# fema-ffrd/gpras

Hardware: AMD Instinct MI355X
Metric: gp_fits_per_sec (higher is better)
Workload: dtype f64; 1 GPU; BASELINE configs[1] as the many-independent-cells workload: exact GP N=4096 d=8 RBF, fit F1 = kernel build + blocked fp64-MFMA Cholesky + alpha + LML, per cell; cells = y columns of one training set with per-cell hyperparameters (the reference's per-mode models); n_train=4096, d=8, kernel=RBF, collective=none (one process), launcher=single process

## Files before the change

### gpras_amd/_lib.py

```python

from __future__ import annotations

import ctypes as C
from pathlib import Path

import numpy as np

import os

LIB_PATH = Path(os.environ["GPRX_LIBRARY"]) if os.environ.get("GPRX_LIBRARY") else Path(__file__).resolve().parent / "libgprx.so"

GPRX_OK, GPRX_EINVAL, GPRX_ENOTPD, GPRX_EHIP, GPRX_ENOMEM, GPRX_ESTATE, GPRX_ERCCL, GPRX_ENOCONV = range(8)
UNIQUE_ID_BYTES = 128
TRAIN_VARIANCE, TRAIN_LENGTHSCALE, TRAIN_NOISE, TRAIN_Z = 1, 2, 4, 8
GEMM_C_LOWER, GEMM_A_LOWER, GEMM_A_UPPER, GEMM_B_LOWER, GEMM_B_UPPER = 1, 2, 4, 8, 16
REDUCE_LOGDET_QUAD, REDUCE_COL, REDUCE_ROWSQ_FINAL, REDUCE_ROW = range(4)

DISTANCE_FORMS = {"difference": 0, "expanded": 1}
KERNEL_IDS = {"RBF": 0, "Matern12": 1, "Matern32": 2, "Matern52": 3, "Exponential": 4}


class GprxLibraryError(RuntimeError):
    """libgprx.so is missing or unusable."""

# ... 142 lines not shown
    "gprx_al_clip_dev": (C.c_int, [_vp, _vp, _i64, _i64, _i64, _i64, _vp, _i64]),
    "gprx_al_timings": (C.c_int, [_vp, _dp]),
    "gprx_dg_create": (C.c_int, [C.c_int, C.POINTER(_vp)]),
    "gprx_dg_destroy": (C.c_int, [_vp]),
    "gprx_dg_last_error": (C.c_char_p, [_vp]),
    "gprx_dg_synchronize": (C.c_int, [_vp]),
    "gprx_dg_sort_u64_dev": (C.c_int, [_vp, _vp, _i64, _vp]),
    "gprx_dg_sort_abs_residual_dev": (C.c_int, [_vp, _vp, _vp, _i64, _vp]),
    "gprx_dg_sort_info": (C.c_int, [_vp, _ip, _dp]),
    "gprx_dg_gather_dev": (C.c_int, [_vp, _vp, _i64, _vp, _i64, _vp]),
    "gprx_dg_scatter_summary_dev": (C.c_int, [_vp, _vp, _vp, _i64, _vp]),
    "gprx_dg_detect_dev": (C.c_int, [_vp, _vp, _vp, _i64, _i64, _vp, _vp, _i64, C.c_double, C.c_int, _vp, C.POINTER(_i64)]),
    "gprx_ev_create": (C.c_int, [C.c_int, _i64, _i64, _i64, _vp, _vp, _vp, _vp, _vp, C.POINTER(_vp)]),
    "gprx_ev_create_empty": (C.c_int, [C.c_int, C.POINTER(_vp)]),
    "gprx_ev_destroy": (C.c_int, [_vp]),
    "gprx_ev_last_error": (C.c_char_p, [_vp]),
    "gprx_ev_synchronize": (C.c_int, [_vp]),
    "gprx_ev_maxima": (C.c_int, [_vp, _vp, _vp, _vp]),
    "gprx_ev_return_periods": (C.c_int, [_vp, _i64, _vp, _vp, _vp]),
    "gprx_ev_rp_eval": (C.c_int, [_vp, C.c_int, _vp, _i64, _vp]),
    "gprx_ev_cov": (C.c_int, [_vp, C.c_int, _vp, _vp]),
    "gprx_ev_eigh": (C.c_int, [_vp, _vp, _vp, _ip]),
    "gprx_ev_scores": (C.c_int, [_vp, C.c_int, C.c_int, _vp]),
    "gprx_ev_standardise": (C.c_int, [_vp, _vp]),
    "gprx_ev_farthest": (C.c_int, [_vp, _vp, _i64, C.c_int, _vp, _i64, _i64, _vp, _vp]),
    "gprx_ev_timings": (C.c_int, [_vp, _dp]),
    "gprx_metrics": (C.c_int, [C.c_int, _vp, _vp, _vp, _i64, _i64, C.c_int, C.c_double, _vp, _vp, _vp, C.POINTER(C.c_uint64)]),
    "gprx_metrics_dev": (C.c_int, [C.c_int, _vp, _vp, _vp, _i64, _i64, C.c_int, C.c_double, _vp, _vp, _vp, C.POINTER(C.c_uint64)]),
    "gprx_kmeans_pp": (C.c_int, [C.c_int, _vp, _i64, C.c_int, _vp, C.c_int, C.c_int, _i64, _vp, _vp]),
    "gprx_kmeans_lloyd": (C.c_int, [C.c_int, _vp, _i64, C.c_int, _vp, C.c_int, C.c_double, C.c_int, _vp, _ip, _ip]),
    "gprx_gather_rows": (C.c_int, [C.c_int, _vp, _i64, _i64, _vp, _vp]),
    "gprx_kmat": (C.c_int, [C.c_int, C.c_int, _vp, _i64, _vp, _i64, C.c_int, _vp, C.c_double, C.c_double, _vp, _i64, _i64, _i64, C.c_int]),
    "gprx_gemm": (C.c_int, [C.c_int, C.c_int, C.c_int, _i64, _i64, _i64, C.c_double, _vp, _i64, _vp, _i64, C.c_double, _vp, _i64, C.c_int, C.c_int]),
    "gprx_potrf": (C.c_int, [C.c_int, _vp, _i64, _i64, _i64, _vp, _ip]),
    "gprx_gemm_batched": (C.c_int, [C.c_int, C.c_int, C.c_int, _i64, _i64, _i64, C.c_double, _vp, _i64, _vp, _i64, C.c_double, _vp, _i64, C.c_int, C.c_int,
                                    C.c_int, _i64, _i64, _i64, C.c_int, _i64, _i64, _i64, _vp, C.c_int, _vp, _i64]),
    "gprx_gemm_splitk": (C.c_int, [C.c_int, C.c_int, C.c_int, _i64, _i64, _i64, C.c_double, _vp, _i64, _vp, _i64, C.c_double, _vp, _i64, _vp, C.c_int,
                                   C.c_int, _i64, _i64, _i64, _i64, _vp, C.c_int]),
    "gprx_trsv_lower": (C.c_int, [C.c_int, _vp, _i64, _vp, _vp, _i64, C.c_int, C.c_int, _i64, _vp]),
    "gprx_potrf_batched": (C.c_int, [C.c_int, _vp, _i64, _i64, _i64, _vp, _vp, _vp, C.c_int, _i64, C.c_int, C.c_int, C.c_int, C.c_int, C.c_int, _ip]),
    "gprx_trsm_lower_left": (C.c_int, [C.c_int, _vp, _i64, _vp, _vp, _i64, _i64, _i64, C.c_int, _i64, _vp]),
    "gprx_trtri_lower": (C.c_int, [C.c_int, _vp, _i64, _vp, _vp, _i64, _vp, _i64, _i64, C.c_int, _i64, _i64, C.c_int]),
    "gprx_transpose_inplace": (C.c_int, [C.c_int, _vp, _i64, _i64, C.c_int, _i64]),
    "gprx_alpha_from_inverse": (C.c_int, [C.c_int, _vp, _i64, _vp, _vp, _vp, _i64, C.c_int, _i64, _i64, _i64]),
    "gprx_reduce_probe": (C.c_int, [C.c_int, C.c_int, _vp, _i64, _vp, _i64, _i64, C.c_double, C.c_double, C.c_int, _vp, C.c_int, _vp, C.c_int, _i64, _i64,
                                    _i64, _i64, _vp, _vp, C.c_int]),
    "gprx_set_tuning": (C.c_int, [C.c_char_p, C.c_int]),
    "gprx_set_handle_tuning": (C.c_int, [_vp, C.c_char_p, C.c_int]),
    "gprx_mfma_f64_peak": (C.c_int, [C.c_int, _dp]),
    "gprx_exp_probe": (C.c_int, [C.c_int, C.c_int, _vp, _i64, _vp]),
}

TUNING_KEYS = (
    "outer_block", "update_tile", "no_lookahead", "split_panel", "dag", "rhs_vector", "cell_kernel", "poison_workspace", "predict_path",
    "sgpr_fused", "sgpr_resident", "wait_handover_us", "sgpr_groups_from", "loeo_blocked_potrf",
    "held_general",
    "pcafit_rowsplit",
)
PCAFIT_ROUTES = ("gram", "covariance")

_lib = None


def load():
    global _lib
    if _lib is not None:
        return _lib
    if not LIB_PATH.exists():
        raise GprxLibraryError(
            f"{LIB_PATH} not found: build it with `python -c 'import __graft_entry__ as g; g.build()'` "
            "(hipcc --offload-arch=gfx950).  gpras_amd has no CPU fallback."
        )
    try:
        lib = C.CDLL(str(LIB_PATH))
    except OSError as exc:
        raise GprxLibraryError(f"cannot load {LIB_PATH}: {exc}") from exc
    for name, (res, args) in PROTOTYPES.items():
        try:
            fn = getattr(lib, name)
        except AttributeError as exc:
            raise GprxLibraryError(f"{LIB_PATH} does not export {name}") from exc
        fn.restype = res
        fn.argtypes = args
    _lib = lib
    return lib


def last_error(handle=None) -> str:
    msg = load().gprx_last_error(handle)
    return msg.decode() if msg else ""


def check(rc: int, handle=None) -> None:
    if rc == GPRX_OK:
        return
    msg = last_error(handle)
    if rc == GPRX_EINVAL:
        raise ValueError(msg)
    if rc == GPRX_ENOTPD:
        raise np.linalg.LinAlgError(msg)
    if rc == GPRX_ENOCONV:
        raise np.linalg.LinAlgError(msg)
    if rc == GPRX_ENOMEM:
        raise MemoryError(msg)
    raise RuntimeError(f"libgprx error {rc}: {msg}")


# ... 44 lines not shown
```

### gpras_amd/csrc/gprx.hip

```cpp
#include "abi_common.h"

#include <algorithm>
#include <chrono>
#include <cmath>
#include <cstdio>
#include <cstdlib>
#include <cstring>
#include <limits>
#include <map>
#include <mutex>
#include <string>
#include <thread>
#include <vector>

#include "gemm_f64.h"
#include "gprx_common.h"
#include "grad.h"
#include "kmat.h"
#include "potrf.h"
#include "potrf_cell.h"
#include "potrf_dag.h"
#include "sgpr.h"
#include "sgpr_asm.h"
#include "sgpr_fused.h"
// ... 622 lines not shown
  });
}

int gprx_trsm_lower_left(int device, const double* l_dev, int64_t lda, const double* inv_diag_dev, double* b_dev, int64_t ldb, int64_t n,
                         int64_t ncols, int cells, int64_t cs, const double* src_dev) {
  return guarded(nullptr, [&]() -> int {
    if (const char* why = solve_probe_invalid(l_dev, lda, inv_diag_dev, n, cells, cs)) return fail(nullptr, GPRX_EINVAL, why);
    if (!b_dev || off16(b_dev) || (src_dev && off16(src_dev))) return fail(nullptr, GPRX_EINVAL, "right-hand side must be given, 16-byte aligned");
    if (ncols <= 0 || ncols > (1 << 30) || ldb < ncols || odd(ldb)) return fail(nullptr, GPRX_EINVAL, "ldb must be even and at least ncols");
    if (src_dev && n != NB) return fail(nullptr, GPRX_EINVAL, "src is for n == 64 only");
    HIPCHK(nullptr, hipSetDevice(device));
    HIPCHK(nullptr, trsm_lower_left(util_stream(), l_dev, lda, inv_diag_dev, b_dev, ldb, (int)n, (int)ncols, cells, cs, src_dev));
    HIPCHK(nullptr, hipStreamSynchronize(util_stream()));
    return GPRX_OK;
  });
}

int gprx_trtri_lower(int device, const double* l_dev, int64_t lda, const double* inv_diag_dev, double* x_dev, int64_t ldx, double* t_dev,
                     int64_t ldt, int64_t np, int cells, int64_t cs_l, int64_t cs_x, int tile) {
  return guarded(nullptr, [&]() -> int {
    if (const char* why = solve_probe_invalid(l_dev, lda, inv_diag_dev, np, cells, cs_l)) return fail(nullptr, GPRX_EINVAL, why);
    if (!x_dev || !t_dev || off16(x_dev) || off16(t_dev)) return fail(nullptr, GPRX_EINVAL, "X and T must be given, 16-byte aligned");
    if (ldx < np || ldt < np || odd(ldx) || odd(ldt) || odd(cs_x) || cs_x < 0) return fail(nullptr, GPRX_EINVAL, "ldx, ldt, cs_x must be even, rows at least np");
    if (tile != 0 && tile != 64 && tile != 128) return fail(nullptr, GPRX_EINVAL, "tile must be 0, 64 or 128");
    HIPCHK(nullptr, hipSetDevice(device));
    HIPCHK(nullptr, trtri_lower(util_stream(), l_dev, lda, inv_diag_dev, x_dev, ldx, t_dev, ldt, (int)np, cells, cs_l, cs_x, tile));
    HIPCHK(nullptr, hipStreamSynchronize(util_stream()));
    return GPRX_OK;
  });
}

int gprx_potrf_batched(int device, double* a_dev, int64_t lda, int64_t np, int64_t extra, double* inv_diag_dev, double* stage_dev,
                       double* yvec_dev, int batch, int64_t cs, int route, int outer_block, int update_tile, int lookahead, int col_base,
                       int* info_host) {
  return guarded(nullptr, [&]() -> int {
    if (!a_dev || !inv_diag_dev || !stage_dev || !info_host) return fail(nullptr, GPRX_EINVAL, "null argument");
    if (np <= 0 || np % NB) return fail(nullptr, GPRX_EINVAL, "np must be a positive multiple of 64");
    if (extra < 0 || np > (1 << 30) || extra > (1 << 30)) return fail(nullptr, GPRX_EINVAL, "extra must not be negative, np and extra at most 2^30");
    if (lda < np || odd(lda) || odd(cs) || cs < 0) return fail(nullptr, GPRX_EINVAL, "lda and cs must be even, lda at least np");
    if (batch > 1 && cs < lda * (np + extra)) return fail(nullptr, GPRX_EINVAL, "cs shorter than one cell's matrix: the cells would overlap");
    if (off16(a_dev) || off16(inv_diag_dev) || off16(stage_dev) || (yvec_dev && off16(yvec_dev)))
      return fail(nullptr, GPRX_EINVAL, "operands must be 16-byte aligned");
    if (batch < 1 || route < 0 || route > 2 || col_base < 0) return fail(nullptr, GPRX_EINVAL, "batch must be positive, route 0, 1 or 2");
    if (yvec_dev && (route != 1 || batch == 1 || extra != 0))
      return fail(nullptr, GPRX_EINVAL, "the vector right-hand side is the split panel's, for batched cells without right-hand-side rows");
    if (route == 2 && extra % NB) return fail(nullptr, GPRX_EINVAL, "the cell kernel takes right-hand-side rows in tiles of 64");
    if (lookahead != 0 && (lookahead != 1 || batch > 1 || route == 2)) return fail(nullptr, GPRX_EINVAL, "look-ahead is for one matrix on routes 0 and 1");
    if (outer_block < 0 || outer_block % NB || (update_tile != 0 && update_tile != 64 && update_tile != 128))
      return fail(nullptr, GPRX_EINVAL, "outer_block must be a multiple of 64, update_tile 0, 64 or 128");
    PotrfTuning tune;
    tune.outer_block = outer_block;
    tune.update_tile = update_tile;
    tune.split_panel = route == 1 ? 1 : -1;
    HIPCHK(nullptr, hipSetDevice(device));
    hipStream_t st = util_stream();
    int* dinfo = nullptr;
    HIPCHK(nullptr, hipMalloc((void**)&dinfo, sizeof(int) * batch));
    hipError_t e = memset_sync(dinfo, 0, sizeof(int) * batch);
    PotrfStreams ps;
    if (e == hipSuccess && lookahead) e = ps.init();
    if (e == hipSuccess)
      e = route == 2 ? potrf_cells(st, a_dev, lda, (int)np, (int)extra, inv_diag_dev, dinfo, batch, cs, 1, col_base)
                     : potrf_lower(st, a_dev, lda, (int)np, (int)extra, inv_diag_dev, dinfo, stage_dev, nullptr, lookahead ? &ps : nullptr, batch, cs, 1,
                                   &tune, col_base, yvec_dev);
    hipError_t e2 = hipStreamSynchronize(st);
    if (ps.aux && e2 == hipSuccess) e2 = hipStreamSynchronize(ps.aux);
    ps.destroy();
    if (e == hipSuccess && e2 == hipSuccess) e2 = copy_sync(info_host, dinfo, sizeof(int) * batch, hipMemcpyDeviceToHost);
    hipFree(dinfo);
    HIPCHK(nullptr, e);
    HIPCHK(nullptr, e2);
    for (int c = 0; c < batch; ++c)
      if (info_host[c]) return fail(nullptr, GPRX_ENOTPD, "matrix not positive definite");
    return GPRX_OK;
  });
}

int gprx_transpose_inplace(int device, double* x_dev, int64_t ld, int64_t n, int cells, int64_t cs) {
  return guarded(nullptr, [&]() -> int {
    if (!x_dev || off16(x_dev)) return fail(nullptr, GPRX_EINVAL, "X must be given, 16-byte aligned");
    if (n <= 0 || n % 64 || n > (1 << 30) || ld < n || odd(ld) || cells < 1 || odd(cs) || cs < 0)
      return fail(nullptr, GPRX_EINVAL, "n must be a positive multiple of 64, ld and cs even");
    HIPCHK(nullptr, hipSetDevice(device));
    HIPCHK(nullptr, transpose_inplace(util_stream(), x_dev, ld, (int)n, cells, cs));
    HIPCHK(nullptr, hipStreamSynchronize(util_stream()));
    return GPRX_OK;
  });
}

int gprx_alpha_from_inverse(int device, const double* x_dev, int64_t ldx, const double* beta_dev, double* part_dev, double* alpha_dev, int64_t np,
                            int cells, int64_t cs_x, int64_t cs_b, int64_t cs_a) {
  return guarded(nullptr, [&]() -> int {
    if (!x_dev || !beta_dev || !part_dev || !alpha_dev) return fail(nullptr, GPRX_EINVAL, "null argument");
    if (np <= 0 || np % NB || np > (1 << 30) || ldx < np || cells < 1 || cs_x < 0 || cs_b < 0 || cs_a < 0)
      return fail(nullptr, GPRX_EINVAL, "np must be a positive multiple of 64");
    HIPCHK(nullptr, hipSetDevice(device));
    HIPCHK(nullptr, alpha_from_inverse(util_stream(), x_dev, ldx, beta_dev, part_dev, alpha_dev, (int)np, cells, cs_x, cs_b, cs_a));
    HIPCHK(nullptr, hipStreamSynchronize(util_stream()));
    return GPRX_OK;
  });
}

int gprx_reduce_probe(int device, int op, const double* m_dev, int64_t ldm, const double* w_dev, int64_t nrows, int64_t ncols, double base,
                      double scale, int accumulate, double* partial_dev, int rows_per_chunk, double* out_dev, int cells, int64_t m_cell,
                      int64_t w_cell, int64_t p_cell, int64_t out_cell, const double* base_tab_dev, const double* base_tab2_dev, int base_stride) {
  return guarded(nullptr, [&]() -> int {
// ... 64 lines not shown
int gprx_panel_acc(unsigned long long* out8, int reset) {
  if (reset) {
    unsigned long long z[8] = {0};
    hipMemcpyToSymbol(HIP_SYMBOL(gprx::g_panel_acc), z, sizeof(z));
  }
  hipMemcpyFromSymbol(out8, HIP_SYMBOL(gprx::g_panel_acc), sizeof(unsigned long long) * 8);
  return 0;
}
#endif
#ifdef GPRX_CELL_ACC
int gprx_cell_acc(unsigned long long* out16, int reset) {
  if (reset) {
    unsigned long long z[16] = {0};
    hipMemcpyToSymbol(HIP_SYMBOL(gprx::g_cell_acc), z, sizeof(z));
  }
  hipMemcpyFromSymbol(out16, HIP_SYMBOL(gprx::g_cell_acc), sizeof(unsigned long long) * 16);
  return 0;
}
#endif
int gprx_sf_stamps(gprx_handle h, int enable, unsigned long long* out) {
  return guarded(h, [&]() -> int {
    if (!h) return fail(h, GPRX_EINVAL, "null handle");
    HIPCHK(h, hipSetDevice(h->device));
    HIPCHK(h, hipStreamSynchronize(h->stream));
    if (out && h->sf_stamps) HIPCHK(h, copy_sync(out, h->sf_stamps, sizeof(unsigned long long) * SF_STAMP_WORDS, hipMemcpyDeviceToHost));
    if (enable && !h->sf_stamps) {
      HIPCHK(h, hipMalloc((void**)&h->sf_stamps, sizeof(unsigned long long) * SF_STAMP_WORDS));
      HIPCHK(h, memset_sync(h->sf_stamps, 0, sizeof(unsigned long long) * SF_STAMP_WORDS));
      drop_graphs(h);
    } else if (!enable && h->sf_stamps) {
      HIPCHK(h, hipFree(h->sf_stamps));
      h->sf_stamps = nullptr;
      drop_graphs(h);
    }
    return GPRX_OK;
  });
}
#ifdef GPRX_PANEL_STAMPS
int gprx_panel_stamps(unsigned long long* out64) {
  hipMemcpyFromSymbol(out64, HIP_SYMBOL(gprx::g_panel_stamps), sizeof(unsigned long long) * 64);
  return 0;
}
#endif

namespace {
bool apply_tuning(PotrfTuning& t, int& predict_path, int& fused, int& resident, const std::string& k, int value) {
  if (k == "outer_block" && value >= 0 && value % 128 == 0) t.outer_block = value;
  else if (k == "update_tile" && (value == 0 || value == 64 || value == 128)) t.update_tile = value;
  else if (k == "no_lookahead") t.no_lookahead = value != 0;
  else if (k == "split_panel" && value >= -1 && value <= 1) t.split_panel = value;
  else if (k == "dag" && value >= -1 && value <= 1) t.dag = value;
  else if (k == "rhs_vector" && value >= -1 && value <= 1) t.rhs_vector = value;
  else if (k == "cell_kernel" && value >= -1 && value <= 1) t.cell_kernel = value;
  else if (k == "poison_workspace" && value >= 0 && value <= 1) t.poison_workspace = value;
  else if (k == "predict_path" && value >= 0 && value <= 2) predict_path = value;
  else if (k == "sgpr_fused" && value >= 0 && value <= 1) fused = value;
  else if (k == "sgpr_resident" && value >= 0 && value <= 1) resident = value;
  else if (k == "wait_handover_us" && value >= 0) wait_handover_us() = value;
  else if (k == "sgpr_groups_from" && value >= 0) sf_groups_from() = value;
  else if (k == "loeo_blocked_potrf" && value >= -1 && value <= 2) loeo_blocked_potrf_force() = value;
  else if (k == "pcafit_rowsplit" && value >= 0 && value <= 1) pcafit_rowsplit_tuning() = value;
  else return false;
  return true;
}
}

int gprx_set_tuning(const char* key, int value) {
  return guarded(nullptr, [&]() -> int {
    if (!key) return fail(nullptr, GPRX_EINVAL, "null key");
    if (!apply_tuning(potrf_tuning(), predict_path_tuning(), sgpr_fused_tuning(), sgpr_resident_tuning(), key, value)) return fail(nullptr, GPRX_EINVAL, "unknown tuning key or bad value");
    return GPRX_OK;
  });
}

int gprx_set_handle_tuning(gprx_handle h, const char* key, int value) {
  return guarded(h, [&]() -> int {
    if (!h || !key) return fail(h, GPRX_EINVAL, "null argument");
    const int fused_before = h->sgpr_fused;
    if (std::string(key) == "held_general") {
      if (value < 0 || value > 1) return fail(h, GPRX_EINVAL, "unknown tuning key or bad value");
      h->held_general = value;
    } else if (!apply_tuning(h->tune, h->predict_path, h->sgpr_fused, h->sgpr_resident, key, value)) {
      return fail(h, GPRX_EINVAL, "unknown tuning key or bad value");
    }
    if (hipSetDevice(h->device) == hipSuccess && hipStreamSynchronize(h->stream) == hipSuccess) drop_graphs(h);
    if (h->sgpr_fused != fused_before) {
      h->sarena_slots = 0;
      if (h->m != 0) h->factorized = false;
    }
    return GPRX_OK;
  });
}

int gprx_mfma_f64_peak(int device, double* tflops) {
  return guarded(nullptr, [&]() -> int {
    if (!tflops) return fail(nullptr, GPRX_EINVAL, "null argument");
    HIPCHK(nullptr, hipSetDevice(device));
    double* out = nullptr;
    HIPCHK(nullptr, hipMalloc((void**)&out, 64));
    hipEvent_t e0, e1;
    hipEventCreate(&e0);
    hipEventCreate(&e1);
    const int iters = 20000, blocks = 256 * 4;
    hipStream_t us = util_stream();
    hipLaunchKernelGGL(mfma_f64_peak_kernel, dim3(blocks), dim3(256), 0, us, out, 100);
    hipEventRecord(e0, us);
// ... 17 lines not shown
```

### gpras_amd/csrc/potrf.h

```cpp
#pragma once
#include <cstdlib>
#include <utility>
#include <vector>

#include "chain64.h"
#include "gemm_f64.h"
#include "gprx_common.h"

namespace gprx {

#ifdef GPRX_PANEL_ACC
__device__ unsigned long long g_panel_acc[8];
#define PACC_DECL unsigned long long pacc_prev_ = 0;
#define PACC(i)                                                                                                       \
  {                                                                                                                   \
    if ((i) == 5) __builtin_amdgcn_s_waitcnt(0);                                                                      \
    const unsigned long long t_ = __builtin_amdgcn_s_memtime();                                                       \
    if (threadIdx.x == 0 && blockIdx.x == 0 && blockIdx.y == 0 && gridDim.x > 2) {                                    \
      if ((i) > 0) atomicAdd(&g_panel_acc[i], t_ - pacc_prev_);                                                       \
      else atomicAdd(&g_panel_acc[0], 1ull);                                                                          \
    }                                                                                                                 \
    pacc_prev_ = t_;                                                                                                  \
  }
#else
// ... 99 lines not shown
  if constexpr (P == 1) { PSTAMP(13) }
  __syncthreads();
  if constexpr (P == 1) { PSTAMP(14) }
  if constexpr (C0 + 8 < NB) {
    constexpr int KT0 = (C0 + 8) / 16;
    double fa[RT][2], fb[4][2];
#pragma unroll
    for (int rt = 0; rt < RT; ++rt)
#pragma unroll
      for (int ks = 0; ks < 2; ++ks) fa[rt][ks] = -c.sX[(WROWS * c.wave + 16 * rt + c.r) * PSUB + 4 * ks + c.g];
#pragma unroll
    for (int kt = KT0; kt < 4; ++kt) {
      const int kk = kt * 16 + c.r;
#pragma unroll
      for (int ks = 0; ks < 2; ++ks) fb[kt][ks] = (kk >= C0 + 8) ? c.sX[kk * PSUB + 4 * ks + c.g] : 0.0;
    }
#pragma unroll
    for (int kt = KT0; kt < 4; ++kt)
#pragma unroll
      for (int rt = 0; rt < RT; ++rt) {
        acc[rt][kt] = __builtin_amdgcn_mfma_f64_16x16x4f64(fa[rt][0], fb[kt][0], acc[rt][kt], 0, 0, 0);
        acc[rt][kt] = __builtin_amdgcn_mfma_f64_16x16x4f64(fa[rt][1], fb[kt][1], acc[rt][kt], 0, 0, 0);
      }
  }
  if ((c.r >> 3) == HALF) {
#pragma unroll
    for (int rt = 0; rt < RT; ++rt)
#pragma unroll
      for (int q = 0; q < 4; ++q) acc[rt][KT][q] = c.sX[(WROWS * c.wave + 16 * rt + c.g + 4 * q) * PSUB + (c.r & 7)];
  }
  if constexpr (P == 1) { PSTAMP(15) }
}

__device__ __forceinline__ void flush_staged_block(const double* __restrict__ prev_stage, double* __restrict__ prev_dst, int64_t lda,
                                                   int prev_pw, int tid) {
  if (!prev_stage) return;
  const int chunks = prev_pw / 2;
  for (int e = tid; e < prev_pw * chunks; e += 256) {
    const int row = e / chunks, cc = e % chunks;
    *reinterpret_cast<d2*>(prev_dst + (int64_t)row * lda + 2 * cc) = *reinterpret_cast<const d2*>(prev_stage + row * prev_pw + 2 * cc);
  }
}

__global__ __launch_bounds__(256) void copy_block_kernel(const double* __restrict__ stage, double* __restrict__ dst, int64_t lda, int pw,
                                                         int64_t cs) {
  flush_staged_block(stage + (int64_t)blockIdx.x * cs, dst + (int64_t)blockIdx.x * cs, lda, pw, threadIdx.x);
}

template <bool FUSE_K64>
__global__ __launch_bounds__(256, 2) void potrf_panel_kernel(double* __restrict__ A, int64_t lda, int rows_below, int nchunks,
                                                          double* __restrict__ inv_diag, int* __restrict__ info, int col0,
                                                          double* __restrict__ stage_out, const double* __restrict__ prev_stage,
                                                          double* __restrict__ prev_dst, int prev_pw, int64_t cs, int info_stride,
                                                          double* __restrict__ yv) {
  constexpr int PWG_ROWS = PANEL_WG_ROWS;
  constexpr int PANEL_ROWS = PANEL_OWN_ROWS;
  constexpr int WROWS = 16 * RT;
#ifndef GPRX_PANEL_NO_SETPRIO
  __builtin_amdgcn_s_setprio(3);
#endif
  {
    const int64_t off = (int64_t)blockIdx.y * cs;
    A += off;
    inv_diag += off;
    stage_out += off;
    if (prev_stage) prev_stage += off;
    if (prev_dst) prev_dst += off;
    info += (int64_t)blockIdx.y * info_stride;
  }
  __shared__ __attribute__((aligned(16))) double sIn[PWG_ROWS * PSUB];
  __shared__ __attribute__((aligned(16))) double sX[PWG_ROWS * PSUB];
  PanelCtx c;
  c.sIn = sIn;
  c.sX = sX;
  c.inv_diag = inv_diag;
  c.tid = threadIdx.x;
  const int lane = c.tid & 63;
  c.wave = c.tid >> 6;
  c.g = lane >> 4;
  c.r = lane & 15;
  c.zero_above = c.tid < NB ? c.tid : (1 << 30);
  c.bad = 0;
  const bool last = (int)blockIdx.x == nchunks;
  c.rinv_out = last ? stage_out + NB * NB : nullptr;
  if (last) flush_staged_block(prev_stage, prev_dst, lda, prev_pw, c.tid);
  c.out = nullptr;
  c.ident = -1;
  if (c.tid < NB) {
    if (last) c.out = stage_out + c.tid * NB;
  } else if (c.tid < PWG_ROWS) {
    if (last && c.tid < 2 * NB) c.ident = c.tid - NB;
  }
  PSTAMP(0)
  PACC_DECL
  PACC(0)

  d4 acc[RT][4];
  {
    const double* rowp[RT][4];
    bool valid[RT][4];
#pragma unroll
    for (int rt = 0; rt < RT; ++rt)
#pragma unroll
      for (int q = 0; q < 4; ++q) {
        const int wrow = WROWS * c.wave + 16 * rt + c.g + 4 * q;
        const int idx = (int)blockIdx.x * PANEL_ROWS + (wrow - NB);
        const bool diag = wrow < NB;
// ... 64 lines not shown
        const int wrow = WROWS * c.wave + 16 * rt + c.g + 4 * q;
#pragma unroll
        for (int kt = 0; kt < 4; ++kt) {
          const int col = kt * 16 + c.r;
          double v = valid[rt][q] ? acc[rt][kt][q] : 0.0;
          if (wrow < NB) {
            v = (col > wrow) ? 0.0 : v;
          } else if (last) {
            v = (col == wrow - NB) ? 1.0 : 0.0;
          }
          acc[rt][kt][q] = v;
        }
      }
  }
  PSTAMP(1)
  PACC(1)

  panel_step<0>(acc, c);
  PSTAMP(2)
  PACC(2)
  panel_step<1>(acc, c);
  panel_step<2>(acc, c);
  panel_step<3>(acc, c);
  PSTAMP(3)
  PACC(3)
  panel_step<4>(acc, c);
  panel_step<5>(acc, c);
  panel_step<6>(acc, c);
  panel_step<7>(acc, c);
  PSTAMP(4)
  PACC(4)
  if (!last) {
#pragma unroll
    for (int rt = 0; rt < RT; ++rt)
#pragma unroll
      for (int q = 0; q < 4; ++q) {
        const int wrow = WROWS * c.wave + 16 * rt + c.g + 4 * q;
        const int idx = (int)blockIdx.x * PANEL_ROWS + (wrow - NB);
        if (wrow >= NB && idx < rows_below) {
          double* dst = A + (int64_t)(NB + idx) * lda + c.r;
#pragma unroll
          for (int kt = 0; kt < 4; ++kt) dst[kt * 16] = acc[rt][kt][q];
        }
      }
  }
  if (last && c.tid == 0 && c.bad != 0) atomicCAS(info, 0, col0 + c.bad);
  if (yv != nullptr && last) {
    yv += (int64_t)blockIdx.y * cs;
    asm volatile("s_waitcnt vmcnt(0)" ::: "memory");
    __syncthreads();
    double* sv = sIn;
    double* sred = sIn + NB;
    static_assert(PWG_ROWS * PSUB >= NB + 256, "the sub-panel buffer holds y_j and the partial sums");
    if (c.tid < NB) sv[c.tid] = yv[c.tid];
    __syncthreads();
    const int a = c.tid & 63, qq = c.tid >> 6;
    const double* row = inv_diag + a * NB + 16 * qq;
    double sum = 0.0;
#pragma unroll
    for (int i = 0; i < 16; ++i) sum = __builtin_fma(row[i], sv[16 * qq + i], sum);
    sred[c.tid] = sum;
    __syncthreads();
    if (c.tid < NB) yv[c.tid] = ((sred[c.tid] + sred[64 + c.tid]) + sred[128 + c.tid]) + sred[192 + c.tid];
  }
  PSTAMP(5)
  PACC(5)
}

constexpr int ROWS_WG = 64 * RT;
__device__ __forceinline__ void wave_sync_lds() {
  __builtin_amdgcn_fence(__ATOMIC_RELEASE, "wavefront");
  __builtin_amdgcn_wave_barrier();
  __builtin_amdgcn_fence(__ATOMIC_ACQUIRE, "wavefront");
}
template <int P>
__device__ __forceinline__ void rows_step(d4 (&acc)[RT][4], double* __restrict__ sIn, double* __restrict__ sX, int tid, int wave, int g, int r,
                                          const double* __restrict__ gstage) {
  constexpr int C0 = 8 * P;
  constexpr int KT = C0 / 16;
  constexpr int HALF = P & 1;
  constexpr int WROWS = 16 * RT;
  if ((r >> 3) == HALF) {
#pragma unroll
    for (int rt = 0; rt < RT; ++rt)
#pragma unroll
      for (int q = 0; q < 4; ++q) sIn[(WROWS * wave + 16 * rt + g + 4 * q) * PSUB + (r & 7)] = acc[rt][KT][q];
  }
  wave_sync_lds();
  const int srow = WROWS * wave + (tid & 63);
  if ((tid & 63) < WROWS) {
    double x[8];
#pragma unroll
    for (int k = 0; k < 8; ++k) {
      double t = sIn[srow * PSUB + k];
#pragma unroll
      for (int m = 0; m < k; ++m) t = __builtin_fma(-x[m], gstage[(C0 + k) * NB + C0 + m], t);
      x[k] = t * gstage[NB * NB + C0 + k];
    }
#pragma unroll
    for (int k = 0; k < 8; ++k) sX[srow * PSUB + k] = x[k];
  }
  wave_sync_lds();
  if constexpr (C0 + 8 < NB) {
    constexpr int KT0 = (C0 + 8) / 16;
    double fa[RT][2], fb[4][2];
#pragma unroll
    for (int rt = 0; rt < RT; ++rt)
#pragma unroll
      for (int ks = 0; ks < 2; ++ks) fa[rt][ks] = -sX[(WROWS * wave + 16 * rt + r) * PSUB + 4 * ks + g];
#pragma unroll
    for (int kt = KT0; kt < 4; ++kt) {
      const int kk = kt * 16 + r;
#pragma unroll
      for (int ks = 0; ks < 2; ++ks) fb[kt][ks] = (kk >= C0 + 8) ? gstage[kk * NB + C0 + 4 * ks + g] : 0.0;
    }
#pragma unroll
    for (int kt = KT0; kt < 4; ++kt)
#pragma unroll
      for (int rt = 0; rt < RT; ++rt) {
        acc[rt][kt] = __builtin_amdgcn_mfma_f64_16x16x4f64(fa[rt][0], fb[kt][0], acc[rt][kt], 0, 0, 0);
        acc[rt][kt] = __builtin_amdgcn_mfma_f64_16x16x4f64(fa[rt][1], fb[kt][1], acc[rt][kt], 0, 0, 0);
      }
  }
  if ((r >> 3) == HALF) {
#pragma unroll
    for (int rt = 0; rt < RT; ++rt)
#pragma unroll
      for (int q = 0; q < 4; ++q) acc[rt][KT][q] = sX[(WROWS * wave + 16 * rt + g + 4 * q) * PSUB + (r & 7)];
  }
}

template <bool FUSE_K64, bool YVEC>
__global__ __launch_bounds__(256, FUSE_K64 ? 2 : 4) void potrf_rows_kernel(double* __restrict__ A21, int64_t lda, int rows_below,
                                                                           const double* __restrict__ stage, int64_t cs, double* __restrict__ yv) {
  constexpr int WG_ROWS = ROWS_WG, WROWS = 16 * RT;
  __shared__ __attribute__((aligned(16))) double sIn[WG_ROWS * PSUB];
  __shared__ __attribute__((aligned(16))) double sX[WG_ROWS * PSUB];
  A21 += (int64_t)blockIdx.y * cs;
  stage += (int64_t)blockIdx.y * cs;
  const int tid = threadIdx.x, lane = tid & 63, wave = tid >> 6, g = lane >> 4, r = lane & 15;
  const int row0 = blockIdx.x * WG_ROWS;
  d4 acc[RT][4];
  {
    const double* rowp[RT][4];
    bool valid[RT][4];
#pragma unroll
    for (int rt = 0; rt < RT; ++rt)
#pragma unroll
      for (int q = 0; q < 4; ++q) {
        const int idx = row0 + WROWS * wave + 16 * rt + g + 4 * q;
        valid[rt][q] = idx < rows_below;
        rowp[rt][q] = A21 + (int64_t)(valid[rt][q] ? idx : 0) * lda + r;
      }
    d4 upd[FUSE_K64 ? RT : 1][4];
    if constexpr (FUSE_K64) {
#pragma unroll
      for (int rt = 0; rt < RT; ++rt)
#pragma unroll
        for (int kt = 0; kt < 4; ++kt) upd[rt][kt] = d4{0.0, 0.0, 0.0, 0.0};
      const double* arow[RT];
#pragma unroll
      for (int rt = 0; rt < RT; ++rt) {
        const int idx = row0 + WROWS * wave + 16 * rt + r;
        arow[rt] = A21 + (int64_t)(idx < rows_below ? idx : 0) * lda - NB + 4 * g;
      }
      const double* brow = A21 - (int64_t)NB * lda + (int64_t)r * lda - NB + 4 * g;
#pragma unroll
      for (int k0 = 0; k0 < NB; k0 += 16) {
        double fa[RT][4], fb[4][4];
#pragma unroll
        for (int rt = 0; rt < RT; ++rt) {
          const d2 lo = *reinterpret_cast<const d2*>(arow[rt] + k0), hi = *reinterpret_cast<const d2*>(arow[rt] + k0 + 2);
          fa[rt][0] = lo.x; fa[rt][1] = lo.y; fa[rt][2] = hi.x; fa[rt][3] = hi.y;
        }
#pragma unroll
        for (int kt = 0; kt < 4; ++kt) {
          const double* bp = brow + (int64_t)(16 * kt) * lda + k0;
          const d2 lo = *reinterpret_cast<const d2*>(bp), hi = *reinterpret_cast<const d2*>(bp + 2);
          fb[kt][0] = lo.x; fb[kt][1] = lo.y; fb[kt][2] = hi.x; fb[kt][3] = hi.y;
        }
#pragma unroll
        for (int j = 0; j < 4; ++j)
#pragma unroll
          for (int rt = 0; rt < RT; ++rt)
#pragma unroll
            for (int kt = 0; kt < 4; ++kt) upd[rt][kt] = __builtin_amdgcn_mfma_f64_16x16x4f64(fa[rt][j], fb[kt][j], upd[rt][kt], 0, 0, 0);
      }
    }
#pragma unroll
    for (int rt = 0; rt < RT; ++rt)
#pragma unroll
      for (int q = 0; q < 4; ++q)
#pragma unroll
        for (int kt = 0; kt < 4; ++kt) acc[rt][kt][q] = rowp[rt][q][kt * 16];
    if constexpr (FUSE_K64) {
#pragma unroll
      for (int rt = 0; rt < RT; ++rt)
#pragma unroll
        for (int kt = 0; kt < 4; ++kt)
#pragma unroll
          for (int q = 0; q < 4; ++q) {
            const double v = -1.0 * upd[rt][kt][q];
            acc[rt][kt][q] = __builtin_fma(1.0, acc[rt][kt][q], v);
          }
    }
#pragma unroll
    for (int rt = 0; rt < RT; ++rt)
#pragma unroll
      for (int q = 0; q < 4; ++q)
#pragma unroll
        for (int kt = 0; kt < 4; ++kt) acc[rt][kt][q] = valid[rt][q] ? acc[rt][kt][q] : 0.0;
  }
  rows_step<0>(acc, sIn, sX, tid, wave, g, r, stage);
  rows_step<1>(acc, sIn, sX, tid, wave, g, r, stage);
  rows_step<2>(acc, sIn, sX, tid, wave, g, r, stage);
  rows_step<3>(acc, sIn, sX, tid, wave, g, r, stage);
  rows_step<4>(acc, sIn, sX, tid, wave, g, r, stage);
  rows_step<5>(acc, sIn, sX, tid, wave, g, r, stage);
  double ybj[YVEC ? 4 : 1], yold[YVEC ? RT : 1][4];
  if constexpr (YVEC) {
    yv += (int64_t)blockIdx.y * cs;
#pragma unroll
    for (int kt = 0; kt < 4; ++kt) ybj[kt] = yv[16 * kt + r];
#pragma unroll
    for (int rt = 0; rt < RT; ++rt)
#pragma unroll
      for (int q = 0; q < 4; ++q) {
        const int idx = row0 + WROWS * wave + 16 * rt + g + 4 * q;
        yold[rt][q] = yv[NB + (idx < rows_below ? idx : 0)];
      }
  }
  rows_step<6>(acc, sIn, sX, tid, wave, g, r, stage);
  rows_step<7>(acc, sIn, sX, tid, wave, g, r, stage);
#pragma unroll
  for (int rt = 0; rt < RT; ++rt)
#pragma unroll
    for (int q = 0; q < 4; ++q) {
      const int idx = row0 + WROWS * wave + 16 * rt + g + 4 * q;
      if (idx < rows_below) {
        double* dst = A21 + (int64_t)idx * lda + r;
#pragma unroll
        for (int kt = 0; kt < 4; ++kt) dst[kt * 16] = acc[rt][kt][q];
      }
    }
  if constexpr (YVEC) {
#pragma unroll
    for (int rt = 0; rt < RT; ++rt)
#pragma unroll
      for (int q = 0; q < 4; ++q) {
        double sum = acc[rt][0][q] * ybj[0];
#pragma unroll
        for (int kt = 1; kt < 4; ++kt) sum = __builtin_fma(acc[rt][kt][q], ybj[kt], sum);
#pragma unroll
        for (int m = 1; m < 16; m <<= 1) sum += __shfl_xor(sum, m, 64);
        const int idx = row0 + WROWS * wave + 16 * rt + g + 4 * q;
        if (r == 0 && idx < rows_below) yv[NB + idx] = yold[rt][q] - sum;
      }
  }
}

constexpr int STAGE_LD = 129;

struct PotrfProfile {
  std::vector<hipEvent_t> pool;
  size_t used = 0;
  std::vector<std::pair<size_t, double>> gemm_marks;
  std::vector<std::pair<size_t, double>> strip_marks;
  std::vector<size_t> panel_marks;
  hipEvent_t next() {
    if (used == pool.size()) {
      hipEvent_t e;
      hipEventCreate(&e);
      pool.push_back(e);
    }
    return pool[used++];
  }
  void reset() {
    used = 0;
    gemm_marks.clear();
    strip_marks.clear();
    panel_marks.clear();
  }
  ~PotrfProfile() {
    for (auto e : pool) hipEventDestroy(e);
  }
};

struct PotrfTuning {
  int outer_block = 0;
  int update_tile = 0;
  int no_lookahead = 0;
  int split_panel = 0;
  int poison_workspace = 0;
  int cell_kernel = 0;
  int rhs_vector = 0;
  int dag = 0;
};
inline PotrfTuning& potrf_tuning() {
  static PotrfTuning t = [] {
    PotrfTuning v;
    if (const char* e = getenv("GPRX_OUTER_BLOCK")) v.outer_block = atoi(e);
    if (const char* e = getenv("GPRX_UPDATE_TILE")) v.update_tile = atoi(e);
    if (const char* e = getenv("GPRX_SPLIT_PANEL")) v.split_panel = atoi(e);
    if (const char* e = getenv("GPRX_DAG")) v.dag = atoi(e);
    if (const char* e = getenv("GPRX_RHS_VECTOR")) v.rhs_vector = atoi(e);
    if (const char* e = getenv("GPRX_CELL_KERNEL")) v.cell_kernel = atoi(e);
    return v;
  }();
  return t;
}

struct PotrfStreams {
  hipStream_t aux = nullptr;
  hipEvent_t block_done = nullptr, tail_done = nullptr;
  hipError_t init() {
    hipError_t e = hipStreamCreateWithFlags(&aux, hipStreamNonBlocking);
    if (e != hipSuccess) return e;
    if ((e = hipEventCreateWithFlags(&block_done, hipEventDisableTiming)) != hipSuccess) return e;
    return hipEventCreateWithFlags(&tail_done, hipEventDisableTiming);
  }
  void destroy() {
    if (aux) hipStreamDestroy(aux);
    if (block_done) hipEventDestroy(block_done);
    if (tail_done) hipEventDestroy(tail_done);
    aux = nullptr;
    block_done = tail_done = nullptr;
  }
};

inline bool potrf_split_panel(const PotrfTuning& tune, int batch) { return tune.split_panel ? tune.split_panel > 0 : batch >= 24; }

inline bool potrf_rhs_vector_ok(const PotrfTuning& tune, int batch) { return tune.rhs_vector >= 0 && batch > 1 && potrf_split_panel(tune, batch); }

inline hipError_t potrf_lower(hipStream_t st, double* A, int64_t lda, int np, int extra, double* inv_diag, int* info,
                              double* diag_stage, PotrfProfile* prof = nullptr, PotrfStreams* ps = nullptr, int batch = 1, int64_t cs = 0,
                              int info_stride = 0, const PotrfTuning* tune_in = nullptr, int col_base = 0, double* yvec = nullptr) {
  const double* prev_stage = nullptr;
  double* prev_dst = nullptr;
  auto mark_gemm = [&](hipStream_t s, int ncols_lower, int rows_rect, int ncols, int k, bool strip = false) {
    if (!prof) return;
    const double elems = 0.5 * (double)ncols_lower * (ncols_lower + 1) + (double)rows_rect * ncols;
    (strip ? prof->strip_marks : prof->gemm_marks).push_back({prof->used, 2.0 * k * elems * batch});
    hipEventRecord(prof->next(), s);
  };
  auto mark_end = [&](hipStream_t s) {
    if (prof) hipEventRecord(prof->next(), s);
  };
  const int total_rows = np + extra;
  const PotrfTuning& tune = tune_in ? *tune_in : potrf_tuning();
  if (tune.no_lookahead) ps = nullptr;
  const int ob = tune.outer_block ? tune.outer_block : (np > 4096 ? 512 : 1024);
  const int bulk_tile = tune.update_tile ? tune.update_tile : 64;
  bool tail_pending = false;
  hipError_t err = hipSuccess;
  const bool split_panel = potrf_split_panel(tune, batch);
  if (yvec && !split_panel) return hipErrorInvalidValue;
  auto panel = [&](int c, bool fuse = false) {
    const int rows_below = total_rows - c - NB;
    double* Acc = A + (int64_t)c * lda + c;
    if (prof) {
      prof->panel_marks.push_back(prof->used);
      hipEventRecord(prof->next(), st);
    }
    double* stage_out = diag_stage + (int64_t)c * STAGE_LD;
    double* invd = inv_diag + (int64_t)(c / NB) * NB * NB;
    double* yv = yvec ? yvec + c : nullptr;
    const int own_rows = split_panel ? 0 : rows_below;
    const int nchunks = (own_rows + PANEL_OWN_ROWS - 1) / PANEL_OWN_ROWS;
    const auto diag = fuse ? potrf_panel_kernel<true> : potrf_panel_kernel<false>;
    hipLaunchKernelGGL(diag, dim3(nchunks + 1, batch), dim3(256), 0, st, Acc, lda,
                       own_rows, nchunks, invd, info, col_base + c, stage_out, prev_stage, prev_dst, NB, cs, info_stride, yv);
    if (split_panel && rows_below > 0) {
      const auto rows = fuse ? (yv ? potrf_rows_kernel<true, true> : potrf_rows_kernel<true, false>)
                             : (yv ? potrf_rows_kernel<false, true> : potrf_rows_kernel<false, false>);
      hipLaunchKernelGGL(rows, dim3((rows_below + ROWS_WG - 1) / ROWS_WG, batch), dim3(256), 0, st, Acc + (int64_t)NB * lda, lda, rows_below,
                         (const double*)stage_out, cs, yv);
    }
    prev_stage = stage_out;
    prev_dst = Acc;
    if (prof) hipEventRecord(prof->next(), st);
  };
  auto update = [&](int c0, int k, int c1, int n, int tile) {
    const int rows = total_rows - c1;
    const double* L21 = A + (int64_t)c1 * lda + c0;
    double* A22 = A + (int64_t)c1 * lda + c1;
    mark_gemm(st, n, rows - n, n, k, k <= 128);
    hipError_t e = launch_gemm(st, 0, 1, rows, n, k, -1.0, L21, lda, L21, lda, 1.0, A22, lda, GEMM_C_LOWER, k == NB ? 64 : tile, batch, cs, cs, cs);
    mark_end(st);
    if (e != hipSuccess && err == hipSuccess) err = e;
  };
  auto factor_range = [&](auto&& self, int c0, int w) -> void {
    if (w <= NB) {
      panel(c0);
      return;
    }
    const int h = ((w / NB + 1) / 2) * NB;
    self(self, c0, h);
    if (h == NB && w - h == NB) {
      panel(c0 + h, true);
      return;
    }
    update(c0, h, c0 + h, w - h, 64);
    self(self, c0 + h, w - h);
  };
  for (int C = 0; C < np; C += ob) {
    const int w = (np - C < ob) ? np - C : ob;
    factor_range(factor_range, C, w);
    if (err != hipSuccess) return err;
    const int R = C + w;
    if (R >= np) break;
    const int wn = (np - R < ob) ? np - R : ob;
    if (ps && tail_pending) hipStreamWaitEvent(st, ps->tail_done, 0);
    update(C, w, R, wn, batch > 1 ? bulk_tile : 64);
    if (err != hipSuccess) return err;
    if (ps) hipEventRecord(ps->block_done, st);
    const int R2 = R + wn;
    if (R2 < np) {
      hipStream_t ts = ps ? ps->aux : st;
      if (ps) hipStreamWaitEvent(ts, ps->block_done, 0);
      const int rows = total_rows - R2, cols = np - R2;
      const double* Lrow = A + (int64_t)R2 * lda + C;
      mark_gemm(ts, cols, rows - cols, cols, w);
      hipError_t e = launch_gemm(ts, 0, 1, rows, cols, w, -1.0, Lrow, lda, Lrow, lda, 1.0, A + (int64_t)R2 * lda + R2, lda, GEMM_C_LOWER,
                                   bulk_tile, batch, cs, cs, cs);
      mark_end(ts);
      if (e != hipSuccess) return e;
      if (ps) {
        hipEventRecord(ps->tail_done, ts);
        tail_pending = true;
      }
    }
  }
  if (prev_stage) hipLaunchKernelGGL(copy_block_kernel, dim3(batch), dim3(256), 0, st, prev_stage, prev_dst, lda, NB, cs);
  if (ps && tail_pending) hipStreamWaitEvent(st, ps->tail_done, 0);
  return hipGetLastError();
}

}
```

Baseline: 2260 fits/s.

## Fuse paired 64-column panel row solves into one rows kernel pass

For batched split-panel Cholesky, two adjacent 64-wide panels are now handled by a paired rows kernel. It runs both triangular row solves in one launch and keeps the y-vector update in LDS between the passes. The first diagonal panel factors its own 64 rows so the second panel can apply the k=64 update, and the rows kernel is refactored into a reusable device function that uses buffer loads and non-temporal loads and stores. This is meant to cut kernel launches and global memory round trips per panel pair. The cost is heavier register pressure, a changed launch-bounds occupancy, and a more complex correctness path.

```diff
diff --git a/gpras_amd/_lib.py b/gpras_amd/_lib.py
--- a/gpras_amd/_lib.py
+++ b/gpras_amd/_lib.py
@@ -218,7 +218,7 @@
 }
 
 TUNING_KEYS = (
-    "outer_block", "update_tile", "no_lookahead", "split_panel", "dag", "rhs_vector", "cell_kernel", "poison_workspace", "predict_path",
+    "outer_block", "update_tile", "no_lookahead", "split_panel", "dag", "rhs_vector", "rows_pair", "cell_kernel", "poison_workspace", "predict_path",
     "sgpr_fused", "sgpr_resident", "wait_handover_us", "sgpr_groups_from", "loeo_blocked_potrf",
     "held_general",
     "pcafit_rowsplit",
diff --git a/gpras_amd/csrc/gprx.hip b/gpras_amd/csrc/gprx.hip
--- a/gpras_amd/csrc/gprx.hip
+++ b/gpras_amd/csrc/gprx.hip
@@ -698,6 +698,7 @@
     tune.outer_block = outer_block;
     tune.update_tile = update_tile;
     tune.split_panel = route == 1 ? 1 : -1;
+    tune.rows_pair = potrf_tuning().rows_pair;
     HIPCHK(nullptr, hipSetDevice(device));
     hipStream_t st = util_stream();
     int* dinfo = nullptr;
@@ -868,6 +869,7 @@
   else if (k == "dag" && value >= -1 && value <= 1) t.dag = value;
   else if (k == "rhs_vector" && value >= -1 && value <= 1) t.rhs_vector = value;
   else if (k == "cell_kernel" && value >= -1 && value <= 1) t.cell_kernel = value;
+  else if (k == "rows_pair" && value >= 0 && value <= 1) t.rows_pair = value;
   else if (k == "poison_workspace" && value >= 0 && value <= 1) t.poison_workspace = value;
   else if (k == "predict_path" && value >= 0 && value <= 2) predict_path = value;
   else if (k == "sgpr_fused" && value >= 0 && value <= 1) fused = value;
diff --git a/gpras_amd/csrc/potrf.h b/gpras_amd/csrc/potrf.h
--- a/gpras_amd/csrc/potrf.h
+++ b/gpras_amd/csrc/potrf.h
@@ -175,7 +175,7 @@
                                                           double* __restrict__ inv_diag, int* __restrict__ info, int col0,
                                                           double* __restrict__ stage_out, const double* __restrict__ prev_stage,
                                                           double* __restrict__ prev_dst, int prev_pw, int64_t cs, int info_stride,
-                                                          double* __restrict__ yv) {
+                                                          double* __restrict__ yv, int y_left) {
   constexpr int PWG_ROWS = PANEL_WG_ROWS;
   constexpr int PANEL_ROWS = PANEL_OWN_ROWS;
   constexpr int WROWS = 16 * RT;
@@ -346,9 +346,20 @@
     double* sv = sIn;
     double* sred = sIn + NB;
     static_assert(PWG_ROWS * PSUB >= NB + 256, "the sub-panel buffer holds y_j and the partial sums");
-    if (c.tid < NB) sv[c.tid] = yv[c.tid];
+    const int a = c.tid & 63, qq = c.tid >> 6;
+    if (FUSE_K64 && y_left) {
+      const double* brow = A + (int64_t)a * lda - NB + 16 * qq;
+      const double* bl = yv - NB + 16 * qq;
+      double sum = 0.0;
+#pragma unroll
+      for (int i = 0; i < 16; ++i) sum = __builtin_fma(brow[i], bl[i], sum);
+      sred[c.tid] = sum;
+      __syncthreads();
+      if (c.tid < NB) sv[c.tid] = yv[c.tid] - (((sred[c.tid] + sred[64 + c.tid]) + sred[128 + c.tid]) + sred[192 + c.tid]);
+    } else {
+      if (c.tid < NB) sv[c.tid] = yv[c.tid];
+    }
     __syncthreads();
-    const int a = c.tid & 63, qq = c.tid >> 6;
     const double* row = inv_diag + a * NB + 16 * qq;
     double sum = 0.0;
 #pragma unroll
@@ -424,27 +435,40 @@
   }
 }
 
-template <bool FUSE_K64, bool YVEC>
-__global__ __launch_bounds__(256, FUSE_K64 ? 2 : 4) void potrf_rows_kernel(double* __restrict__ A21, int64_t lda, int rows_below,
-                                                                           const double* __restrict__ stage, int64_t cs, double* __restrict__ yv) {
-  constexpr int WG_ROWS = ROWS_WG, WROWS = 16 * RT;
-  __shared__ __attribute__((aligned(16))) double sIn[WG_ROWS * PSUB];
-  __shared__ __attribute__((aligned(16))) double sX[WG_ROWS * PSUB];
-  A21 += (int64_t)blockIdx.y * cs;
-  stage += (int64_t)blockIdx.y * cs;
-  const int tid = threadIdx.x, lane = tid & 63, wave = tid >> 6, g = lane >> 4, r = lane & 15;
-  const int row0 = blockIdx.x * WG_ROWS;
+__device__ __forceinline__ d2 ld2_l2(__amdgpu_buffer_rsrc_t rs, unsigned voff, unsigned soff) {
+  typedef unsigned int u4v __attribute__((ext_vector_type(4)));
+  const u4v v = __builtin_amdgcn_raw_buffer_load_b128(rs, voff, soff, 16);
+  d2 out;
+  __builtin_memcpy(&out, &v, 16);
+  return out;
+}
+template <int M>
+__device__ __forceinline__ double lane_xor(double v) {
+  int w[2];
+  __builtin_memcpy(w, &v, 8);
+  w[0] = __builtin_amdgcn_ds_swizzle(w[0], (M << 10) | 0x1f);
+  w[1] = __builtin_amdgcn_ds_swizzle(w[1], (M << 10) | 0x1f);
+  __builtin_memcpy(&v, w, 8);
+  return v;
+}
+template <bool FUSE_K64, bool YVEC, bool X_L2, bool Y_IN, bool Y_OUT, bool NT_IN = false, bool NT_OUT = false>
+__device__ __forceinline__ void rows_pass(double* __restrict__ A21, int64_t lda, int rows_below, int row0, const double* __restrict__ stage,
+                                          double* __restrict__ yv, int64_t ycell, int ybeta, int yrows, double* __restrict__ sIn,
+                                          double* __restrict__ sX) {
+  constexpr int WROWS = 16 * RT;
+  const int lane = __lane_id(), wave = __builtin_amdgcn_readfirstlane(threadIdx.x >> 6), tid = 64 * wave + lane, g = lane >> 4, r = lane & 15;
   d4 acc[RT][4];
   {
-    const double* rowp[RT][4];
+    const char* wg0 = reinterpret_cast<const char*>(A21 + (int64_t)row0 * lda);
+    unsigned rowp[RT][4];
     bool valid[RT][4];
 #pragma unroll
     for (int rt = 0; rt < RT; ++rt)
 #pragma unroll
       for (int q = 0; q < 4; ++q) {
-        const int idx = row0 + WROWS * wave + 16 * rt + g + 4 * q;
-        valid[rt][q] = idx < rows_below;
-        rowp[rt][q] = A21 + (int64_t)(valid[rt][q] ? idx : 0) * lda + r;
+        const int lrow = WROWS * wave + 16 * rt + g + 4 * q;
+        valid[rt][q] = row0 + lrow < rows_below;
+        rowp[rt][q] = ((unsigned)(valid[rt][q] ? lrow : 0) * (unsigned)lda + r) * 8u;
       }
     d4 upd[FUSE_K64 ? RT : 1][4];
     if constexpr (FUSE_K64) {
@@ -453,10 +477,14 @@
 #pragma unroll
         for (int kt = 0; kt < 4; ++kt) upd[rt][kt] = d4{0.0, 0.0, 0.0, 0.0};
       const double* arow[RT];
+      [[maybe_unused]] __amdgpu_buffer_rsrc_t xrs;
+      [[maybe_unused]] unsigned xoff[RT];
+      if constexpr (X_L2) xrs = __builtin_amdgcn_make_buffer_rsrc(A21 + (int64_t)row0 * lda - NB, 0, 0xffffffff, 0x00020000);
 #pragma unroll
       for (int rt = 0; rt < RT; ++rt) {
         const int idx = row0 + WROWS * wave + 16 * rt + r;
         arow[rt] = A21 + (int64_t)(idx < rows_below ? idx : 0) * lda - NB + 4 * g;
+        if constexpr (X_L2) xoff[rt] = ((unsigned)(idx < rows_below ? idx - row0 : 0) * (unsigned)lda + 4u * g) * 8u;
       }
       const double* brow = A21 - (int64_t)NB * lda + (int64_t)r * lda - NB + 4 * g;
 #pragma unroll
@@ -464,7 +492,14 @@
         double fa[RT][4], fb[4][4];
 #pragma unroll
         for (int rt = 0; rt < RT; ++rt) {
-          const d2 lo = *reinterpret_cast<const d2*>(arow[rt] + k0), hi = *reinterpret_cast<const d2*>(arow[rt] + k0 + 2);
+          d2 lo, hi;
+          if constexpr (X_L2) {
+            lo = ld2_l2(xrs, xoff[rt], 8u * k0);
+            hi = ld2_l2(xrs, xoff[rt], 8u * k0 + 16u);
+          } else {
+            lo = *reinterpret_cast<const d2*>(arow[rt] + k0);
+            hi = *reinterpret_cast<const d2*>(arow[rt] + k0 + 2);
+          }
           fa[rt][0] = lo.x; fa[rt][1] = lo.y; fa[rt][2] = hi.x; fa[rt][3] = hi.y;
         }
 #pragma unroll
@@ -486,7 +521,10 @@
 #pragma unroll
       for (int q = 0; q < 4; ++q)
 #pragma unroll
-        for (int kt = 0; kt < 4; ++kt) acc[rt][kt][q] = rowp[rt][q][kt * 16];
+        for (int kt = 0; kt < 4; ++kt) {
+          const double* src = reinterpret_cast<const double*>(wg0 + rowp[rt][q] + kt * 128);
+          acc[rt][kt][q] = NT_IN ? __builtin_nontemporal_load(src) : *src;
+        }
     if constexpr (FUSE_K64) {
 #pragma unroll
       for (int rt = 0; rt < RT; ++rt)
@@ -512,16 +550,18 @@
   rows_step<4>(acc, sIn, sX, tid, wave, g, r, stage);
   rows_step<5>(acc, sIn, sX, tid, wave, g, r, stage);
   double ybj[YVEC ? 4 : 1], yold[YVEC ? RT : 1][4];
+  [[maybe_unused]] int yrow0 = row0;
   if constexpr (YVEC) {
-    yv += (int64_t)blockIdx.y * cs;
-#pragma unroll
-    for (int kt = 0; kt < 4; ++kt) ybj[kt] = yv[16 * kt + r];
+    yv += ycell;
+    asm volatile("" : "+s"(yrow0));
+#pragma unroll
+    for (int kt = 0; kt < 4; ++kt) ybj[kt] = yv[ybeta + 16 * kt + r];
 #pragma unroll
     for (int rt = 0; rt < RT; ++rt)
 #pragma unroll
       for (int q = 0; q < 4; ++q) {
-        const int idx = row0 + WROWS * wave + 16 * rt + g + 4 * q;
-        yold[rt][q] = yv[NB + (idx < rows_below ? idx : 0)];
+        const int idx = yrow0 + WROWS * wave + 16 * rt + g + 4 * q;
+        yold[rt][q] = Y_IN ? sIn[(WROWS * wave + 16 * rt + g + 4 * q) * PSUB + 8] : yv[yrows + (idx < rows_below ? idx : 0)];
       }
   }
   rows_step<6>(acc, sIn, sX, tid, wave, g, r, stage);
@@ -534,7 +574,10 @@
       if (idx < rows_below) {
         double* dst = A21 + (int64_t)idx * lda + r;
 #pragma unroll
-        for (int kt = 0; kt < 4; ++kt) dst[kt * 16] = acc[rt][kt][q];
+        for (int kt = 0; kt < 4; ++kt) {
+          if constexpr (NT_OUT) __builtin_nontemporal_store(acc[rt][kt][q], dst + kt * 16);
+          else dst[kt * 16] = acc[rt][kt][q];
+        }
       }
     }
   if constexpr (YVEC) {
@@ -545,12 +588,43 @@
         double sum = acc[rt][0][q] * ybj[0];
 #pragma unroll
         for (int kt = 1; kt < 4; ++kt) sum = __builtin_fma(acc[rt][kt][q], ybj[kt], sum);
-#pragma unroll
-        for (int m = 1; m < 16; m <<= 1) sum += __shfl_xor(sum, m, 64);
-        const int idx = row0 + WROWS * wave + 16 * rt + g + 4 * q;
-        if (r == 0 && idx < rows_below) yv[NB + idx] = yold[rt][q] - sum;
-      }
-  }
+        sum += lane_xor<1>(sum);
+        sum += lane_xor<2>(sum);
+        sum += lane_xor<4>(sum);
+        sum += lane_xor<8>(sum);
+        const int idx = yrow0 + WROWS * wave + 16 * rt + g + 4 * q;
+        if constexpr (Y_OUT) {
+          if (r == 0) sIn[(WROWS * wave + 16 * rt + g + 4 * q) * PSUB + 8] = yold[rt][q] - sum;
+        } else {
+          if (r == 0 && idx < rows_below) yv[yrows + idx] = yold[rt][q] - sum;
+        }
+      }
+  }
+}
+
+template <bool FUSE_K64, bool YVEC>
+__global__ __launch_bounds__(256, FUSE_K64 ? 3 : 4) void potrf_rows_kernel(double* __restrict__ A21, int64_t lda, int rows_below,
+                                                                           const double* __restrict__ stage, int64_t cs, double* __restrict__ yv) {
+  __shared__ __attribute__((aligned(16))) double sIn[ROWS_WG * PSUB];
+  __shared__ __attribute__((aligned(16))) double sX[ROWS_WG * PSUB];
+  const int64_t off = (int64_t)blockIdx.y * cs;
+  rows_pass<FUSE_K64, YVEC, false, false, false>(A21 + off, lda, rows_below, blockIdx.x * ROWS_WG, stage + off, yv, off, 0, NB, sIn, sX);
+}
+
+template <bool YVEC>
+__global__ __launch_bounds__(256, 3) void potrf_rows_pair_kernel(double* __restrict__ A21, int64_t lda, int rows_below,
+                                                                 const double* __restrict__ stage, const double* __restrict__ stage2, int64_t cs,
+                                                                 double* __restrict__ yv) {
+  __shared__ __attribute__((aligned(16))) double sIn[ROWS_WG * PSUB];
+  __shared__ __attribute__((aligned(16))) double sX[ROWS_WG * PSUB];
+  const int64_t off = (int64_t)blockIdx.y * cs;
+  const int row0 = blockIdx.x * ROWS_WG;
+  rows_pass<false, YVEC, false, false, true, true, false>(A21 + off, lda, rows_below, row0, stage + off, yv, off, 0, 2 * NB, sIn, sX);
+  asm volatile("s_waitcnt vmcnt(0)" ::: "memory");
+  wave_sync_lds();
+  int row0b = row0;
+  asm volatile("" : "+s"(row0b));
+  rows_pass<true, YVEC, true, true, false, true, true>(A21 + off + NB, lda, rows_below, row0b, stage2 + off, yv, off, NB, 2 * NB, sIn, sX);
 }
 
 constexpr int STAGE_LD = 129;
@@ -589,6 +663,7 @@
   int cell_kernel = 0;
   int rhs_vector = 0;
   int dag = 0;
+  int rows_pair = 1;
 };
 inline PotrfTuning& potrf_tuning() {
   static PotrfTuning t = [] {
@@ -599,6 +674,7 @@
     if (const char* e = getenv("GPRX_DAG")) v.dag = atoi(e);
     if (const char* e = getenv("GPRX_RHS_VECTOR")) v.rhs_vector = atoi(e);
     if (const char* e = getenv("GPRX_CELL_KERNEL")) v.cell_kernel = atoi(e);
+    if (const char* e = getenv("GPRX_ROWS_PAIR")) v.rows_pair = atoi(e) != 0;
     return v;
   }();
   return t;
@@ -649,7 +725,8 @@
   hipError_t err = hipSuccess;
   const bool split_panel = potrf_split_panel(tune, batch);
   if (yvec && !split_panel) return hipErrorInvalidValue;
-  auto panel = [&](int c, bool fuse = false) {
+  const bool rows_pair = split_panel && batch > 1 && tune.rows_pair != 0;
+  auto panel = [&](int c, bool fuse = false, int pair = 0) {
     const int rows_below = total_rows - c - NB;
     double* Acc = A + (int64_t)c * lda + c;
     if (prof) {
@@ -659,12 +736,18 @@
     double* stage_out = diag_stage + (int64_t)c * STAGE_LD;
     double* invd = inv_diag + (int64_t)(c / NB) * NB * NB;
     double* yv = yvec ? yvec + c : nullptr;
-    const int own_rows = split_panel ? 0 : rows_below;
+    const int own_rows = split_panel ? (pair == 1 ? NB : 0) : rows_below;
     const int nchunks = (own_rows + PANEL_OWN_ROWS - 1) / PANEL_OWN_ROWS;
     const auto diag = fuse ? potrf_panel_kernel<true> : potrf_panel_kernel<false>;
     hipLaunchKernelGGL(diag, dim3(nchunks + 1, batch), dim3(256), 0, st, Acc, lda,
-                       own_rows, nchunks, invd, info, col_base + c, stage_out, prev_stage, prev_dst, NB, cs, info_stride, yv);
-    if (split_panel && rows_below > 0) {
+                       own_rows, nchunks, invd, info, col_base + c, stage_out, prev_stage, prev_dst, NB, cs, info_stride, yv, (int)(pair == 2 && yv));
+    if (pair == 2) {
+      if (rows_below > 0) {
+        const auto rows = yv ? potrf_rows_pair_kernel<true> : potrf_rows_pair_kernel<false>;
+        hipLaunchKernelGGL(rows, dim3((rows_below + ROWS_WG - 1) / ROWS_WG, batch), dim3(256), 0, st, Acc + (int64_t)NB * lda - NB, lda, rows_below,
+                           (const double*)(stage_out - (int64_t)NB * STAGE_LD), (const double*)stage_out, cs, yv ? yv - NB : nullptr);
+      }
+    } else if (split_panel && rows_below > 0 && pair == 0) {
       const auto rows = fuse ? (yv ? potrf_rows_kernel<true, true> : potrf_rows_kernel<true, false>)
                              : (yv ? potrf_rows_kernel<false, true> : potrf_rows_kernel<false, false>);
       hipLaunchKernelGGL(rows, dim3((rows_below + ROWS_WG - 1) / ROWS_WG, batch), dim3(256), 0, st, Acc + (int64_t)NB * lda, lda, rows_below,
@@ -689,6 +772,11 @@
       return;
     }
     const int h = ((w / NB + 1) / 2) * NB;
+    if (h == NB && w - h == NB && rows_pair) {
+      panel(c0, false, 1);
+      panel(c0 + h, true, 2);
+      return;
+    }
     self(self, c0, h);
     if (h == NB && w - h == NB) {
       panel(c0 + h, true);
```

New measurement: 2283 fits/s (median of 6 runs). 1.0% higher.
